# leggedrobotics/delora

Hardware: AMD Instinct MI355X
Metric: training scan-pairs/sec, KITTI 64x2048 range images (higher is better)
Workload: dtype f32; 1 GPU; KITTI-shaped 64x2048, batch=8 pairs/GPU, raw scans of ~141k points (ragged, raster order), steps rotate over 8 distinct HBM-resident batches, online normals, ResNet pose CNN (11.9M params, identity-pretrained state), Adam; BASELINE configs[1]; global_batch=8, parallelism=dp1, cnn=fp32, cnn_impl=hip trunk: fp32 MFMA, fused Winograd F(2x2,3x3) + direct implicit GEMM, channels_last=False, hip_graph=False, distinct_batches=8, priming_steps=8

## Files before the change

### delora_amd/_lib.py

```python
import ctypes
import os

_HERE = os.path.dirname(os.path.abspath(__file__))
LIB_PATH = os.path.join(_HERE, "csrc", "libdelora_hip.so")
ABI_VERSION = 10


class DeloraHipError(RuntimeError):
    pass


class SensorStruct(ctypes.Structure):
    _fields_ = [("H", ctypes.c_int32), ("W", ctypes.c_int32),
                ("hfov0", ctypes.c_double), ("hfov1", ctypes.c_double),
                ("vfov0", ctypes.c_double), ("vfov1", ctypes.c_double)]


_vp, _i32, _i64, _u32, _f32, _sz = (ctypes.c_void_p, ctypes.c_int32, ctypes.c_int64, ctypes.c_uint32,
                                    ctypes.c_float, ctypes.c_size_t)
_SP = ctypes.POINTER(SensorStruct)

SIGNATURES = {
    "dl_abi_version": (_i32, []),
    "dl_last_error": (ctypes.c_char_p, []),
# ... 70 lines not shown
    "dl_heads_single_bwd_workspace_bytes": (_sz, [_i32, _i32, _i32, _i32, _i32, _i32, _i32]),
    "dl_heads_single_bwd": (_i32, [_vp, _vp, _i32, _i32, _i32, _i32, _i32, _i32, _i32, _i32, _vp, _vp, _vp, _vp, _vp, _vp, _vp, _vp, _vp, _vp]),
    "dl_dropout_scale_f32": (_i32, [_vp, _u32, ctypes.c_double, _i64, _vp, _vp]),
    "dl_stem_input_nhwc_drop_f32": (_i32, [_vp, _i32, _i32, _i32, _i32, _vp, ctypes.c_double, _vp, _vp]),
    "dl_channel_scale_nhwc_t": (_i32, [_vp, _vp, _i32, _i32, _i32, _i32, _vp, _vp]),
    "dl_channel_scale_bwd_act_nhwc_t": (_i32, [_vp, _vp, _vp, _i32, _i32, _i32, _i32, _i32, _vp, _vp]),
    "dl_tower_wide_drop_f32": (_i32, [_vp, _vp, ctypes.c_double, _i32, _i32, _i32, _i32, _i32, _vp, _vp]),
    "dl_tower_wide_drop_bwd_f32": (_i32, [_vp, _vp, _vp, ctypes.c_double, _i32, _i32, _i32, _i32, _i32, _i32, _vp, _vp]),
    "dl_mean_hw_nhwc_h": (_i32, [_vp, _i32, _i32, _i32, _i32, _vp, _vp]),
    "dl_mean_hw_bwd_act_h": (_i32, [_vp, _vp, _i32, _i32, _i32, _i32, _i32, _vp, _vp]),
    "dl_conv2d_wgrad_h_workspace_bytes": (_sz, [_i32, _i32, _i32, _i32, _i32, _i32, _i32, _i32]),
    "dl_conv2d_wgrad_nhwc_h": (_i32, [_vp, _vp, _vp, _vp, _i32, _i32, _i32, _i32, _i32, _i32, _i32, _i32, _i32, _vp]),
    "dl_wgrad_batch_plan": (_i64, [_vp, _vp, _i32, _i32, _i32, _vp]),
    "dl_wino_wgrad3x3_batch_workspace_bytes": (_sz, [_vp, _i32]),
    "dl_wino_wgrad3x3_batch_nhwc_f32": (_i32, [_vp, _i32, _vp, _vp]),
    "dl_conv2d_wgrad_batch_workspace_bytes": (_sz, [_vp, _i32]),
    "dl_conv2d_wgrad_batch_nhwc_f32": (_i32, [_vp, _i32, _vp, _vp]),
    "dl_conv2d_wgrad_batch_h_workspace_bytes": (_sz, [_vp, _i32]),
    "dl_conv2d_wgrad_batch_nhwc_h": (_i32, [_vp, _i32, _vp, _i32, _vp]),
    "dl_conv_plan_describe": (_i32, [_i32, _i32, _i32, _i32, _i32, _i32, _i32, _i32, _i32, _i32, _i32, _i32, ctypes.c_char_p, _sz]),
    "dl_pose_net_prepared_bytes": (_sz, [_vp, _i32, _i32, _i32]),
    "dl_pose_net_prepare": (_i32, [_vp, _i32, _i32, _i32, _vp, _vp]),
    "dl_pose_net_workspace_bytes": (_sz, [_vp, _i32, _i32, _i32]),
    "dl_pose_net_forward": (_i32, [_vp, _vp, _vp, _i64, _vp, _i64, _i32, _i32, _i32, _vp, _vp, _vp, _vp, _vp]),
    "dl_odometry_workspace_bytes": (_sz, [_vp, _SP, _i32, _i32, _i32]),
    "dl_odometry_push": (_i32, [_vp, _vp, _SP, _vp, _i64, _i32, _vp, _vp, _vp, _vp, _vp, _vp, _vp, _vp]),
    "dl_profile_begin": (_i32, [_i32, ctypes.c_char_p]),
    "dl_profile_end": (_i32, [_vp, _i32, ctypes.POINTER(ctypes.c_int32), ctypes.POINTER(ctypes.c_int32)]),
    "dl_profile_pause": (_i32, [_i32]),
}
# ... 109 lines not shown
```

### delora_amd/csrc/wino.hip

```cpp
#include "common.h"
#include <cstdlib>

typedef float f32x16 __attribute__((ext_vector_type(16)));
typedef float f32x4 __attribute__((ext_vector_type(4)));
typedef float f32x2 __attribute__((ext_vector_type(2)));
typedef int i32x4 __attribute__((ext_vector_type(4)));

#define WN_THREADS 512
#define WN_CK 8
#define WN_KB 64
#define WN_TILES 64
#define WN_PLANE (WN_TILES * WN_CK + 16)
#define WN_EPI_ADD 1u
#define WN_EPI_ACT 2u
#define WN_EPI_DACT 4u

struct WinoArgs {
  const float* x;
  const float* u;
  float* y;
  const float* add;
  const float* dsrc;
  int N, H, W, C, K;
  int act;
// ... 518 lines not shown
template <bool NEG> __device__ __forceinline__ f32x2 w3_g01(f32x2 h, f32x2 c01) {
  f32x2 r;
  if (NEG) asm volatile("v_pk_fma_f32 %0, %1, %2, %1 op_sel:[1,0,0] op_sel_hi:[1,1,0] neg_lo:[1,0,1] neg_hi:[1,0,1]" : "=v"(r) : "v"(h), "s"(c01));
  else asm volatile("v_pk_fma_f32 %0, %1, %2, %1 op_sel:[1,0,0] op_sel_hi:[1,1,0]" : "=v"(r) : "v"(h), "s"(c01));
  return r;
}
template <bool NEG> __device__ __forceinline__ f32x2 w3_g23(f32x2 h, f32x2 c10) {
  f32x2 r;
  if (NEG) asm volatile("v_pk_fma_f32 %0, %1, %2, %1 op_sel:[0,0,1] op_sel_hi:[0,1,1] neg_lo:[1,0,0] neg_hi:[1,0,0]" : "=v"(r) : "v"(h), "s"(c10));
  else asm volatile("v_pk_fma_f32 %0, %1, %2, %1 op_sel:[0,0,1] op_sel_hi:[0,1,1] neg_lo:[0,0,1] neg_hi:[0,0,1]" : "=v"(r) : "v"(h), "s"(c10));
  return r;
}

struct W3Pos { int n, ta, b8; };

__device__ __forceinline__ void wino_wgrad_body3(const WWArgs& a, const int blk) {
  static_assert((2 * W3_BUF + W3_RAW + W3_GRAW) * 4 <= 163840, "LDS budget");
  __shared__ __attribute__((aligned(16))) float lds[2 * W3_BUF + W3_RAW + W3_GRAW];
  float* raw = lds + 2 * W3_BUF;
  float* graw = raw + W3_RAW;
  const int tid = threadIdx.x, lane = tid & 63, wave = __builtin_amdgcn_readfirstlane(tid >> 6);
  const int li = lane & 31, half = lane >> 5;
  const int mb = wave & 1, nb = (wave >> 1) & 1, xh = wave >> 2;
  const int CT = a.C / 64;
  int t = blk;
  const int slab = t % a.nslabs; t /= a.nslabs;
  const int ct = t % CT;
  const int kt = t / CT;
  const int k0 = kt * 64, c0 = ct * 64;
  const int th = a.H / 2, tw8 = (a.W / 2) / 8;
  const int total_chunks = a.N * th * tw8;
  const int ch_begin = slab * a.chunks_per_slab;
  const int ch_end = min(ch_begin + a.chunks_per_slab, total_chunks);
  if (ch_begin >= ch_end) return;

  const unsigned lds_base = (unsigned)(__SIZE_TYPE__)((__attribute__((address_space(3))) char*)lds);
  const int tp = wave & 3;
#define W3_SWZ(R) ((((R) >> 2) & 1) | (((((R) >> 1) ^ ((R) >> 3)) & 1) << 1))
  const int w_off = lane * 16 + ((tp ^ W3_SWZ(lane)) * 4);
  const float* rsrc = (xh == 0 ? raw : graw) + (4 * tp) * 64 + lane;
  const unsigned voff_x = (unsigned)((lane >> 4) * a.C * 4 + (lane & 15) * 16);
  const unsigned voff_g = (unsigned)((lane >> 4) * a.K * 4 + (lane & 15) * 16);
  const unsigned voff_l = (unsigned)(((lane >> 4) == 0 ? a.W - 1 : (lane >> 4) - 1) * a.C * 4 + (lane & 15) * 16);
  const unsigned voff_r = (unsigned)(((lane >> 4) == 0 ? a.W - 1 : 0) * a.C * 4 + (lane & 15) * 16);
// ... 52 lines not shown
#define W3_DMASK()          { if (top) { _Pragma("unroll") for (int j = 0; j < 6; ++j) P[0][j][0] = 0.f; }                        \
                              if (bot) { _Pragma("unroll") for (int j = 0; j < 6; ++j) P[1][j][1] = 0.f; } }
#define W3_DT(E, RP, B)     { constexpr int o_ = 2 * (E);                                                                           \
                              T[RP][B] = (B) == 0 ? P[RP][o_] - P[RP][o_ + 2] : (B) == 1 ? P[RP][o_ + 1] + P[RP][o_ + 2]               \
                                       : (B) == 2 ? P[RP][o_ + 2] - P[RP][o_ + 1] : P[RP][o_ + 1] - P[RP][o_ + 3]; }
#define W3_DV(E, B)         { V01[E][B] = w3_v01(T[0][B], T[1][B]); V23[E][B] = w3_v23(T[0][B], T[1][B]); }
#define W3_WR(OPER, B)      { f32x4 lo_ = {V01[0][B][0], V01[0][B][1], V01[1][B][0], V01[1][B][1]};                                  \
                              f32x4 hi_ = {V23[0][B][0], V23[0][B][1], V23[1][B][0], V23[1][B][1]};                                  \
                              *reinterpret_cast<f32x4*>(nxt + (OPER) + (B) * W3_PLANE + w_off) = lo_;                                \
                              *reinterpret_cast<f32x4*>(nxt + (OPER) + (4 + (B)) * W3_PLANE + w_off) = hi_; }
#define W3_GLD()            W3_RD2(P[0][0], 0, 16) W3_RD2(P[0][1], 1, 17) W3_RD2(P[0][2], 2, 18) W3_RD2(P[0][3], 3, 19)
#define W3_GH(E)            { T[E][1] = P[0][2 * (E)] + P[0][2 * (E) + 1]; T[E][2] = P[0][2 * (E)] - P[0][2 * (E) + 1]; }
#define W3_GV(E, B)         { if ((B) == 0) { V01[E][0] = w3_g01<false>(P[0][2 * (E)], c01); V23[E][0] = w3_g23<false>(P[0][2 * (E)], c10); }              \
                              else if ((B) == 3) { V01[E][3] = w3_g01<true>(P[0][2 * (E) + 1], c01); V23[E][3] = w3_g23<true>(P[0][2 * (E) + 1], c10); } \
                              else { V01[E][B] = w3_g01<false>(T[E][B], c01); V23[E][B] = w3_g23<false>(T[E][B], c10); } }

#define W3_FR_FROM(HP, BP)                                                                                                \
  {                                                                                                                       \
    av[(HP) & 1] = *reinterpret_cast<const f32x4*>((BP) + ((HP) >> 1) * W3_PLANE + (((HP) & 1) ? a_off1 : a_off0));       \
    bv[(HP) & 1] = *reinterpret_cast<const f32x4*>((BP) + ((HP) >> 1) * W3_PLANE + (((HP) & 1) ? b_off1 : b_off0));       \
  }
#define W3_FR(HP) W3_FR_FROM(HP, cur)
#define W3_M(HP, J, ...)                                                                                                  \
  {                                                                                                                       \
    acc[((J) & 1) * 4 + ((HP) >> 1)] = __builtin_amdgcn_mfma_f32_32x32x2f32(av[(HP) & 1][J], bv[(HP) & 1][J], acc[((J) & 1) * 4 + ((HP) >> 1)], 0, 0, 0); \
    asm volatile("" : "+v"(acc[((J) & 1) * 4 + ((HP) >> 1)]) :: "memory");                                                 \
    __builtin_amdgcn_sched_barrier(0);                                                                                    \
    __VA_ARGS__                                                                                                           \
    __builtin_amdgcn_sched_barrier(0);                                                                                    \
  }
// ... 3 lines not shown
    int u = ch_begin;
    p1.b8 = u % tw8; u /= tw8;
    p1.ta = u % th;
    p1.n = u / th;
  }
  dma(p1);
  asm volatile("s_waitcnt vmcnt(0)" ::: "memory");
  __syncthreads();
  {
    float* nxt = lds;
    const bool top = p1.ta == 0, bot = p1.ta == th - 1;
    if (xh == 0) {
      W3_DLD_0A() W3_DLD_0B() W3_DLD_1A() W3_DLD_1B()
      asm volatile("s_waitcnt lgkmcnt(0)" ::: "memory");
      W3_DMASK()
      W3_DT(0, 0, 0) W3_DT(0, 0, 1) W3_DT(0, 0, 2) W3_DT(0, 0, 3) W3_DT(0, 1, 0) W3_DT(0, 1, 1) W3_DT(0, 1, 2) W3_DT(0, 1, 3)
      W3_DV(0, 0) W3_DV(0, 1) W3_DV(0, 2) W3_DV(0, 3)
      W3_DT(1, 0, 0) W3_DT(1, 0, 1) W3_DT(1, 0, 2) W3_DT(1, 0, 3) W3_DT(1, 1, 0) W3_DT(1, 1, 1) W3_DT(1, 1, 2) W3_DT(1, 1, 3)
      W3_DV(1, 0) W3_DV(1, 1) W3_DV(1, 2) W3_DV(1, 3)
      W3_WR(W3_OPER, 0) W3_WR(W3_OPER, 1) W3_WR(W3_OPER, 2) W3_WR(W3_OPER, 3)
    } else {
      W3_GLD()
      asm volatile("s_waitcnt lgkmcnt(0)" ::: "memory");
      W3_GH(0) W3_GH(1)
      W3_GV(0, 0) W3_GV(0, 1) W3_GV(0, 2) W3_GV(0, 3) W3_GV(1, 0) W3_GV(1, 1) W3_GV(1, 2) W3_GV(1, 3)
      W3_WR(0, 0) W3_WR(0, 1) W3_WR(0, 2) W3_WR(0, 3)
    }
  }
  __syncthreads();
  if (ch_begin + 1 < ch_end) advance(p1);
  dma(p1);
  asm volatile("s_waitcnt vmcnt(0)" ::: "memory");
  __syncthreads();

  f32x4 av[2], bv[2];
  {
    const float* cur = lds;
    W3_FR(0)
  }
#define W3_TAIL()                                                                                                         \
    W3_M(6, 0, W3_FR(7)) W3_M(6, 1, ) W3_M(6, 2, ) W3_M(6, 3, )                                                           \
    asm volatile("s_waitcnt vmcnt(0) lgkmcnt(0)" ::: "memory");                                                           \
    __builtin_amdgcn_s_barrier();                                                                                         \
    __builtin_amdgcn_sched_barrier(0);                                                                                    \
    W3_M(7, 0, W3_FR_FROM(0, nxt)) W3_M(7, 1, ) W3_M(7, 2, ) W3_M(7, 3, )
#define W3_BAR_M()                                                                                                        \
    asm volatile("s_waitcnt lgkmcnt(0)" ::: "memory");                                                                    \
    __builtin_amdgcn_s_barrier();                                                                                         \
    __builtin_amdgcn_sched_barrier(0);
  if (xh == 0) {
    for (int ch = ch_begin; ch < ch_end; ++ch) {
      const float* cur = lds + ((ch - ch_begin) & 1) * W3_BUF;
      float* nxt = lds + ((ch - ch_begin + 1) & 1) * W3_BUF;
      const bool top = p1.ta == 0, bot = p1.ta == th - 1;
      W3Pos p2 = p1;
      if (ch + 2 < ch_end) advance(p2);
      W3_M(0, 0, WW_IF_FR(W3_FR(1)) WW_IF_T(W3_DLD_0A())) W3_M(0, 1, WW_IF_T(W3_DLD_0B())) W3_M(0, 2, WW_IF_T(W3_DLD_1A())) W3_M(0, 3, WW_IF_T(W3_DLD_1B()))
      W3_M(1, 0, WW_IF_FR(W3_FR(2))) W3_M(1, 1, ) W3_M(1, 2, ) W3_M(1, 3, )
      asm volatile("s_waitcnt lgkmcnt(0)" ::: "memory");
      WW_IF_BAR(__builtin_amdgcn_s_barrier();)
      __builtin_amdgcn_sched_barrier(0);
      W3_M(2, 0, WW_IF_FR(W3_FR(3)) WW_IF_DMA(dma(p2);)) W3_M(2, 1, WW_IF_T(W3_DMASK()) WW_IF_T(W3_DT(0, 0, 0)) WW_IF_T(W3_DT(0, 0, 1))) W3_M(2, 2, WW_IF_T(W3_DT(0, 0, 2)) WW_IF_T(W3_DT(0, 0, 3))) W3_M(2, 3, WW_IF_T(W3_DT(0, 1, 0)) WW_IF_T(W3_DT(0, 1, 1)))
      W3_M(3, 0, WW_IF_FR(W3_FR(4)) WW_IF_T(W3_DT(0, 1, 2)) WW_IF_T(W3_DT(0, 1, 3))) W3_M(3, 1, WW_IF_T(W3_DV(0, 0))) W3_M(3, 2, WW_IF_T(W3_DV(0, 1))) W3_M(3, 3, WW_IF_T(W3_DV(0, 2)))
      W3_M(4, 0, WW_IF_FR(W3_FR(5)) WW_IF_T(W3_DV(0, 3))) W3_M(4, 1, WW_IF_T(W3_DT(1, 0, 0)) WW_IF_T(W3_DT(1, 0, 1))) W3_M(4, 2, WW_IF_T(W3_DT(1, 0, 2)) WW_IF_T(W3_DT(1, 0, 3))) W3_M(4, 3, WW_IF_T(W3_DT(1, 1, 0)) WW_IF_T(W3_DT(1, 1, 1)))
      W3_M(5, 0, WW_IF_FR(W3_FR(6)) WW_IF_T(W3_DT(1, 1, 2)) WW_IF_T(W3_DT(1, 1, 3))) W3_M(5, 1, WW_IF_T(W3_DV(1, 0)) WW_IF_T(W3_WR(W3_OPER, 0))) W3_M(5, 2, WW_IF_T(W3_DV(1, 1)) WW_IF_T(W3_WR(W3_OPER, 1))) W3_M(5, 3, WW_IF_T(W3_DV(1, 2)) WW_IF_T(W3_WR(W3_OPER, 2)))
// ... 33 lines not shown
#undef W3_RD2
#undef W3_DLD_0A
#undef W3_DLD_0B
#undef W3_DLD_1A
#undef W3_DLD_1B
#undef W3_DMASK
#undef W3_DT
#undef W3_DV
#undef W3_WR
#undef W3_GLD
#undef W3_GH
#undef W3_GV
#undef W3_FR
#undef W3_FR_FROM
#undef W3_M
  float* wp = a.ws + ((size_t)slab * 16) * a.K * a.C;
#pragma unroll
  for (int xl = 0; xl < 8; ++xl) {
    const int xi = xh * 8 + xl;
#pragma unroll
    for (int q = 0; q < 16; ++q) {
      const int m = mb * 32 + 8 * (q / 4) + 4 * half + (q % 4);
      wp[((size_t)xi * a.K + k0 + m) * a.C + c0 + nb * 32 + li] = acc[xl][q];
    }
  }
}

template <bool RAG>
__global__ __launch_bounds__(WW_THREADS) void k_wino_wgrad(WWArgs a) {
#ifndef WW_OLD
  if constexpr (!RAG) wino_wgrad_body3(a, blockIdx.x);
  else
#endif
  wino_wgrad_body<RAG>(a, blockIdx.x);
}

struct WWBatchArgs {
  WWArgs layer[DL_WGRAD_BATCH];
  int first_wg[DL_WGRAD_BATCH + 1];
  int n;
};
template <bool RAG>
__global__ __launch_bounds__(WW_THREADS) void k_wino_wgrad_batch(WWBatchArgs b) {
  int l = 0;
#pragma unroll
  for (int i = 1; i < DL_WGRAD_BATCH; ++i)
    if (i < b.n && (int)blockIdx.x >= b.first_wg[i]) l = i;
  const WWArgs a = b.layer[l];
#ifndef WW_OLD
  if constexpr (!RAG) wino_wgrad_body3(a, (int)blockIdx.x - b.first_wg[l]);
  else
#endif
  wino_wgrad_body<RAG>(a, (int)blockIdx.x - b.first_wg[l]);
}

__device__ __forceinline__ void wino_wgrad_sum_body(const float* __restrict__ ws, int nslabs, size_t count4, float* __restrict__ u, size_t i) {
  if (i >= count4) return;
  f32x4 s = {0.f, 0.f, 0.f, 0.f};
  for (int sl = 0; sl < nslabs; ++sl) s += reinterpret_cast<const f32x4*>(ws)[(size_t)sl * count4 + i];
  reinterpret_cast<f32x4*>(u)[i] = s;
}
__global__ __launch_bounds__(256) void k_wino_wgrad_sum(const float* __restrict__ ws, int nslabs, size_t count4, float* __restrict__ u) {
  wino_wgrad_sum_body(ws, nslabs, count4, u, (size_t)blockIdx.x * 256 + threadIdx.x);
}

__device__ __forceinline__ void wino_wgrad_out_body(const float* __restrict__ uu, int K, int C, float* __restrict__ dw, size_t i);
__global__ __launch_bounds__(256) void k_wino_wgrad_out(const float* __restrict__ uu, int K, int C, float* __restrict__ dw) {
  wino_wgrad_out_body(uu, K, C, dw, (size_t)blockIdx.x * 256 + threadIdx.x);
// ... 194 lines not shown
    if (it.a.nslabs > 1) {
      sum.src[sum.n] = it.a.ws; sum.dst[sum.n] = it.usum; sum.K[sum.n] = it.a.K; sum.C[sum.n] = it.a.C; sum.nslabs[sum.n] = it.a.nslabs;
      sum.first_block[sum.n] = sum_blocks;
      sum_blocks += (int)(((size_t)16 * it.a.K * it.a.C / 4 + 255) / 256);
      ++sum.n;
    }
    out.src[out.n] = it.usum; out.dst[out.n] = it.dw; out.K[out.n] = it.a.K; out.C[out.n] = it.a.C;
    out.first_block[out.n] = out_blocks;
    out_blocks += (int)(((size_t)it.a.K * it.a.C + 255) / 256);
    ++out.n;
  }
  sum.first_block[sum.n] = sum_blocks; out.first_block[out.n] = out_blocks;
  if (sum.n) DL_LAUNCH_PLAIN(k_wino_wgrad_sum_batch, dim3(sum_blocks), dim3(256), st, sum);
  DL_LAUNCH_PLAIN(k_wino_wgrad_out_batch, dim3(out_blocks), dim3(256), st, out);
  return dl_check_launch("dl_wino_wgrad3x3_batch_nhwc_f32");
}

__global__ __launch_bounds__(256) void k_wino_split_sum(const float* __restrict__ part, int splits, size_t count4, float* __restrict__ y,
                                                         const float* __restrict__ add, const float* __restrict__ dsrc, int act, unsigned epi) {
  const size_t i = (size_t)blockIdx.x * 256 + threadIdx.x;
  if (i >= count4) return;
  const f32x4* p = reinterpret_cast<const f32x4*>(part) + i;
  f32x4 v = p[0];
  for (int s = 1; s < splits; ++s) v += p[(size_t)s * count4];
  if (epi & WN_EPI_ADD) v += reinterpret_cast<const f32x4*>(add)[i];
  if (epi & WN_EPI_ACT) {
    if (act == 1) { v[0] = dl_tanh(v[0]); v[1] = dl_tanh(v[1]); v[2] = dl_tanh(v[2]); v[3] = dl_tanh(v[3]); }
    else { v[0] = wn_act(v[0], act); v[1] = wn_act(v[1], act); v[2] = wn_act(v[2], act); v[3] = wn_act(v[3], act); }
  }
  if (epi & WN_EPI_DACT) {
// ... 193 lines not shown
```

### delora_amd/models/ring_conv.py

```python
import ctypes
import os

import torch

from .. import _lib

ACT = {"none": 0, "tanh": 1, "relu": 2}
USE_WINOGRAD = True
EPI_ADD, EPI_ACT, EPI_DACT, EPI_ADD_GRID = 1, 2, 4, 8


def _ptr(t):
    return ctypes.c_void_p(t.data_ptr()) if t is not None else ctypes.c_void_p(0)


def _stream():
    return ctypes.c_void_p(torch.cuda.current_stream().cuda_stream)


ALLOC_SKEW = 0
_skew_state = {"i": 0}


def _empty(shape, dtype, device):
# ... 76 lines not shown
    lib = _lib.load()
    out = []
    for i0 in range(0, len(items), _lib.WGRAD_BATCH):
        part = items[i0:i0 + _lib.WGRAD_BATCH]
        arr, dws = _wgrad_layer_table(part)
        ap = ctypes.cast(arr, ctypes.c_void_p)
        nbytes = getattr(lib, size_fn)(ap, len(part))
        if not nbytes:
            raise _lib.DeloraHipError(what + ": " + (lib.dl_last_error() or b"").decode())
        ws = torch.empty((nbytes // 4,), dtype=torch.float32, device=part[0][0].device)
        _lib.check(getattr(lib, run_fn)(ap, len(part), _ptr(ws), *extra, _stream()), what)
        out += dws
    return out


def wgrad_batch(items):
    wino, direct = [], []
    for i, (x, g, ks, stride) in enumerate(items):
        N, H, W, C = x.shape
        K = g.shape[3]
        if (USE_WINOGRAD_WGRAD and ks == 3 and tuple(stride) == (1, 1) and C >= WINO_WGRAD_MIN_C_BATCHED and C % 64 == 0 and K % 64 == 0 and W >= 2
                and N * H * W * max(C, K) < 2 ** 31 and H * W * max(C, K) < 2 ** 30):
            wino.append(i)
        else:
            direct.append(i)
    out = [None] * len(items)
    if wino:
        for i, dw in zip(wino, _wgrad_batch_call([items[i] for i in wino], "dl_wino_wgrad3x3_batch_workspace_bytes", "dl_wino_wgrad3x3_batch_nhwc_f32",
                                                 "dl_wino_wgrad3x3_batch_nhwc_f32")):
            out[i] = dw
    if direct:
        for i, dw in zip(direct, _wgrad_batch_call([items[i] for i in direct], "dl_conv2d_wgrad_batch_workspace_bytes", "dl_conv2d_wgrad_batch_nhwc_f32",
                                                   "dl_conv2d_wgrad_batch_nhwc_f32")):
            out[i] = dw
    return out


def wino_ok(H, W, C, K):
    return H >= 1 and W >= 1 and C % 8 == 0 and K % 64 == 0


# ... 844 lines not shown
```

### include/delora_hip.h

```cpp
#ifndef DELORA_HIP_H
#define DELORA_HIP_H

#include <stddef.h>
#include <stdint.h>

#ifdef __cplusplus
extern "C" {
#endif

#define DL_ABI_VERSION 10

typedef void* dl_stream;

typedef enum {
  DL_OK = 0,
  DL_ERR_INVALID_ARGUMENT = -1,
  DL_ERR_LAUNCH = -2,
  DL_ERR_UNSUPPORTED = -3
} dl_status;

typedef struct {
  int32_t H;
  int32_t W;
  double hfov0, hfov1;
// ... 146 lines not shown
int dl_wino_wgrad3x3_nhwc_f32(const float* x, const float* g, float* dw, void* workspace, int32_t N, int32_t H, int32_t W,
                              int32_t C, int32_t K, dl_stream stream);

#define DL_WGRAD_BATCH 24
typedef struct dl_wgrad_layer {
  const void* x;
  const void* g;
  float* dw;
  int32_t N, H, W, C, K, ksize, stride_h, stride_w;
} dl_wgrad_layer;
int64_t dl_wgrad_batch_plan(const int32_t* tiles, const int32_t* chunks, int32_t n, int32_t slots, int32_t partial_cost, int32_t* nslabs);
size_t dl_wino_wgrad3x3_batch_workspace_bytes(const dl_wgrad_layer* layers, int32_t n);
int dl_wino_wgrad3x3_batch_nhwc_f32(const dl_wgrad_layer* layers, int32_t n, void* workspace, dl_stream stream);
size_t dl_conv2d_wgrad_batch_workspace_bytes(const dl_wgrad_layer* layers, int32_t n);
int dl_conv2d_wgrad_batch_nhwc_f32(const dl_wgrad_layer* layers, int32_t n, void* workspace, dl_stream stream);

int dl_conv_weights_h(const float* w, void* w_fwd, void* w_bwd, int32_t K, int32_t taps, int32_t C, int32_t dtype, dl_stream stream);
#define DL_CONVH_BATCH 32
typedef struct {
  const float* w;
  void* w_fwd;
  void* w_bwd;
  int32_t K, taps, C;
} dl_convh_layer;
int dl_conv_weights_batch_h(const dl_convh_layer* layers, int32_t n, int32_t dtype, dl_stream stream);
int dl_conv2d_nhwc_h(const void* x, const void* w, void* y, const void* add, const void* dsrc, int32_t N, int32_t H, int32_t W,
                     int32_t C, int32_t K, int32_t ksize, int32_t stride_h, int32_t stride_w, int32_t transposed, int32_t dtype,
                     int32_t act, uint32_t epilogue, dl_stream stream);
int dl_conv2d_dgrad_strided_nhwc_h(const void* g, const void* w, void* dx, const void* add_grid, const void* dsrc, int32_t N,
                                   int32_t H, int32_t W, int32_t K, int32_t C, int32_t ksize, int32_t stride_h, int32_t stride_w,
// ... 127 lines not shown
```

Before: 693.6 scan-pairs/s.

## Add Winograd weight-gradient path for stride-(1,2) 3x3 convolutions via column polyphase split

Adds a batched Winograd F(2x2,3x3) weight-gradient kernel for 3x3 convolutions with stride (1,2). The input is treated as two interleaved polyphase halves of width W/2 and 2C channels, and only the live Winograd column sets are computed (three for the odd phase, two for the even phase). A templated body skips the dead columns with its own MFMA/transform schedules, followed by a slab-sum kernel and an output kernel that folds the two phases back into 3x3 filter taps. Python routes eligible strided layers to this path instead of the direct implicit-GEMM wgrad, aiming to cut MFMA work and memory traffic. The cost is extra workspace, an extra reduction/combine launch and more code complexity.

```diff
diff --git a/delora_amd/_lib.py b/delora_amd/_lib.py
--- a/delora_amd/_lib.py
+++ b/delora_amd/_lib.py
@@ -108,6 +108,9 @@
     "dl_wgrad_batch_plan": (_i64, [_vp, _vp, _i32, _i32, _i32, _vp]),
     "dl_wino_wgrad3x3_batch_workspace_bytes": (_sz, [_vp, _i32]),
     "dl_wino_wgrad3x3_batch_nhwc_f32": (_i32, [_vp, _i32, _vp, _vp]),
+    "dl_wino_strided_wgrad_takes": (_i32, [_i32, _i32, _i32, _i32, _i32, _i32, _i32]),
+    "dl_wino_strided_wgrad3x3_batch_workspace_bytes": (_sz, [_vp, _i32]),
+    "dl_wino_strided_wgrad3x3_batch_nhwc_f32": (_i32, [_vp, _i32, _vp, _vp]),
     "dl_conv2d_wgrad_batch_workspace_bytes": (_sz, [_vp, _i32]),
     "dl_conv2d_wgrad_batch_nhwc_f32": (_i32, [_vp, _i32, _vp, _vp]),
     "dl_conv2d_wgrad_batch_h_workspace_bytes": (_sz, [_vp, _i32]),
diff --git a/delora_amd/csrc/wino.hip b/delora_amd/csrc/wino.hip
--- a/delora_amd/csrc/wino.hip
+++ b/delora_amd/csrc/wino.hip
@@ -556,20 +556,23 @@
 
 struct W3Pos { int n, ta, b8; };
 
-__device__ __forceinline__ void wino_wgrad_body3(const WWArgs& a, const int blk) {
-  static_assert((2 * W3_BUF + W3_RAW + W3_GRAW) * 4 <= 163840, "LDS budget");
-  __shared__ __attribute__((aligned(16))) float lds[2 * W3_BUF + W3_RAW + W3_GRAW];
+static_assert((2 * W3_BUF + W3_RAW + W3_GRAW) * 4 <= 163840, "LDS budget");
+__shared__ __attribute__((aligned(16))) float w3_lds[2 * W3_BUF + W3_RAW + W3_GRAW];
+template <int LIVE, bool UPPER = LIVE == 0x7>
+__device__ __forceinline__ void wino_wgrad_body3_live(const WWArgs& a, const int blk) {
+  static_assert(LIVE == 0xF || LIVE == 0x7 || LIVE == 0x6, "column sets with a schedule");
+  float* const lds = w3_lds;
   float* raw = lds + 2 * W3_BUF;
   float* graw = raw + W3_RAW;
   const int tid = threadIdx.x, lane = tid & 63, wave = __builtin_amdgcn_readfirstlane(tid >> 6);
   const int li = lane & 31, half = lane >> 5;
   const int mb = wave & 1, nb = (wave >> 1) & 1, xh = wave >> 2;
-  const int CT = a.C / 64;
+  const int CT = LIVE == 0xF ? a.C / 64 : a.C / 128;
   int t = blk;
   const int slab = t % a.nslabs; t /= a.nslabs;
   const int ct = t % CT;
   const int kt = t / CT;
-  const int k0 = kt * 64, c0 = ct * 64;
+  const int k0 = kt * 64, c0 = ct * 64 + (UPPER ? a.C / 2 : 0);
   const int th = a.H / 2, tw8 = (a.W / 2) / 8;
   const int total_chunks = a.N * th * tw8;
   const int ch_begin = slab * a.chunks_per_slab;
@@ -652,6 +655,13 @@
 #define W3_GV(E, B)         { if ((B) == 0) { V01[E][0] = w3_g01<false>(P[0][2 * (E)], c01); V23[E][0] = w3_g23<false>(P[0][2 * (E)], c10); }              \
                               else if ((B) == 3) { V01[E][3] = w3_g01<true>(P[0][2 * (E) + 1], c01); V23[E][3] = w3_g23<true>(P[0][2 * (E) + 1], c10); } \
                               else { V01[E][B] = w3_g01<false>(T[E][B], c01); V23[E][B] = w3_g23<false>(T[E][B], c10); } }
+#define W3_B(B, ...)        { if constexpr ((LIVE >> (B)) & 1) { __VA_ARGS__ } }
+#define W3_DLD7_0A() W3_RD2(P[0][0], 0, 20) W3_RD2(P[0][1], 1, 21) W3_RD2(P[0][2], 2, 22)
+#define W3_DLD7_1A() W3_RD2(P[1][0], 40, 60) W3_RD2(P[1][1], 41, 61) W3_RD2(P[1][2], 42, 62)
+#define W3_DLD6_0A() W3_RD2(P[0][1], 1, 21) W3_RD2(P[0][2], 2, 22)
+#define W3_DLD6_1A() W3_RD2(P[1][1], 41, 61) W3_RD2(P[1][2], 42, 62)
+#define W3_DLDL_0B() W3_RD2(P[0][3], 3, 23) W3_RD2(P[0][4], 4, 24)
+#define W3_DLDL_1B() W3_RD2(P[1][3], 43, 63) W3_RD2(P[1][4], 44, 64)
 
 #define W3_FR_FROM(HP, BP)                                                                                                \
   {                                                                                                                       \
@@ -685,17 +695,20 @@
       W3_DLD_0A() W3_DLD_0B() W3_DLD_1A() W3_DLD_1B()
       asm volatile("s_waitcnt lgkmcnt(0)" ::: "memory");
       W3_DMASK()
-      W3_DT(0, 0, 0) W3_DT(0, 0, 1) W3_DT(0, 0, 2) W3_DT(0, 0, 3) W3_DT(0, 1, 0) W3_DT(0, 1, 1) W3_DT(0, 1, 2) W3_DT(0, 1, 3)
-      W3_DV(0, 0) W3_DV(0, 1) W3_DV(0, 2) W3_DV(0, 3)
-      W3_DT(1, 0, 0) W3_DT(1, 0, 1) W3_DT(1, 0, 2) W3_DT(1, 0, 3) W3_DT(1, 1, 0) W3_DT(1, 1, 1) W3_DT(1, 1, 2) W3_DT(1, 1, 3)
-      W3_DV(1, 0) W3_DV(1, 1) W3_DV(1, 2) W3_DV(1, 3)
-      W3_WR(W3_OPER, 0) W3_WR(W3_OPER, 1) W3_WR(W3_OPER, 2) W3_WR(W3_OPER, 3)
+      W3_B(0, W3_DT(0, 0, 0)) W3_B(1, W3_DT(0, 0, 1)) W3_B(2, W3_DT(0, 0, 2)) W3_B(3, W3_DT(0, 0, 3))
+      W3_B(0, W3_DT(0, 1, 0)) W3_B(1, W3_DT(0, 1, 1)) W3_B(2, W3_DT(0, 1, 2)) W3_B(3, W3_DT(0, 1, 3))
+      W3_B(0, W3_DV(0, 0)) W3_B(1, W3_DV(0, 1)) W3_B(2, W3_DV(0, 2)) W3_B(3, W3_DV(0, 3))
+      W3_B(0, W3_DT(1, 0, 0)) W3_B(1, W3_DT(1, 0, 1)) W3_B(2, W3_DT(1, 0, 2)) W3_B(3, W3_DT(1, 0, 3))
+      W3_B(0, W3_DT(1, 1, 0)) W3_B(1, W3_DT(1, 1, 1)) W3_B(2, W3_DT(1, 1, 2)) W3_B(3, W3_DT(1, 1, 3))
+      W3_B(0, W3_DV(1, 0)) W3_B(1, W3_DV(1, 1)) W3_B(2, W3_DV(1, 2)) W3_B(3, W3_DV(1, 3))
+      W3_B(0, W3_WR(W3_OPER, 0)) W3_B(1, W3_WR(W3_OPER, 1)) W3_B(2, W3_WR(W3_OPER, 2)) W3_B(3, W3_WR(W3_OPER, 3))
     } else {
       W3_GLD()
       asm volatile("s_waitcnt lgkmcnt(0)" ::: "memory");
       W3_GH(0) W3_GH(1)
-      W3_GV(0, 0) W3_GV(0, 1) W3_GV(0, 2) W3_GV(0, 3) W3_GV(1, 0) W3_GV(1, 1) W3_GV(1, 2) W3_GV(1, 3)
-      W3_WR(0, 0) W3_WR(0, 1) W3_WR(0, 2) W3_WR(0, 3)
+      W3_B(0, W3_GV(0, 0)) W3_B(1, W3_GV(0, 1)) W3_B(2, W3_GV(0, 2)) W3_B(3, W3_GV(0, 3))
+      W3_B(0, W3_GV(1, 0)) W3_B(1, W3_GV(1, 1)) W3_B(2, W3_GV(1, 2)) W3_B(3, W3_GV(1, 3))
+      W3_B(0, W3_WR(0, 0)) W3_B(1, W3_WR(0, 1)) W3_B(2, W3_WR(0, 2)) W3_B(3, W3_WR(0, 3))
     }
   }
   __syncthreads();
@@ -704,10 +717,11 @@
   asm volatile("s_waitcnt vmcnt(0)" ::: "memory");
   __syncthreads();
 
+  constexpr int HP0 = LIVE & 1 ? 0 : 2;
   f32x4 av[2], bv[2];
   {
     const float* cur = lds;
-    W3_FR(0)
+    W3_FR(HP0)
   }
 #define W3_TAIL()                                                                                                         \
     W3_M(6, 0, W3_FR(7)) W3_M(6, 1, ) W3_M(6, 2, ) W3_M(6, 3, )                                                           \
@@ -719,7 +733,81 @@
     asm volatile("s_waitcnt lgkmcnt(0)" ::: "memory");                                                                    \
     __builtin_amdgcn_s_barrier();                                                                                         \
     __builtin_amdgcn_sched_barrier(0);
-  if (xh == 0) {
+#define W3_BAR_E()                                                                                                        \
+    asm volatile("s_waitcnt vmcnt(0) lgkmcnt(0)" ::: "memory");                                                           \
+    __builtin_amdgcn_s_barrier();                                                                                         \
+    __builtin_amdgcn_sched_barrier(0);
+  if constexpr (LIVE != 0xF) {
+    if (xh == 0) { if constexpr (LIVE == 0x7) { W3_DLD7_0A() W3_DLD7_1A() } else { W3_DLD6_0A() W3_DLD6_1A() } W3_DLDL_0B() W3_DLDL_1B() }
+    else { W3_GLD() }
+  }
+  if constexpr (LIVE == 0x7) {
+    if (xh == 0) {
+      for (int ch = ch_begin; ch < ch_end; ++ch) {
+        const float* cur = lds + ((ch - ch_begin) & 1) * W3_BUF;
+        float* nxt = lds + ((ch - ch_begin + 1) & 1) * W3_BUF;
+        const bool top = p1.ta == 0, bot = p1.ta == th - 1;
+        W3Pos p2 = p1;
+        if (ch + 2 < ch_end) advance(p2);
+        W3_BAR_M()
+        W3_M(0, 0, W3_FR(1) dma(p2);) W3_M(0, 1, W3_DMASK() W3_DT(0, 0, 0) W3_DT(0, 0, 1)) W3_M(0, 2, W3_DT(0, 0, 2) W3_DT(0, 1, 0)) W3_M(0, 3, W3_DT(0, 1, 1) W3_DT(0, 1, 2))
+        W3_M(1, 0, W3_FR(2) W3_DV(0, 0)) W3_M(1, 1, W3_DV(0, 1)) W3_M(1, 2, W3_DV(0, 2)) W3_M(1, 3, W3_DT(1, 0, 0) W3_DT(1, 0, 1))
+        W3_M(2, 0, W3_FR(3) W3_DT(1, 0, 2)) W3_M(2, 1, W3_DT(1, 1, 0) W3_DT(1, 1, 1)) W3_M(2, 2, W3_DT(1, 1, 2)) W3_M(2, 3, W3_DV(1, 0))
+        W3_M(3, 0, W3_FR(4) W3_WR(W3_OPER, 0)) W3_M(3, 1, W3_DV(1, 1)) W3_M(3, 2, W3_WR(W3_OPER, 1)) W3_M(3, 3, W3_DV(1, 2))
+        W3_M(4, 0, W3_FR(5) W3_WR(W3_OPER, 2)) W3_M(4, 1, ) W3_M(4, 2, ) W3_M(4, 3, )
+        W3_BAR_E()
+        W3_M(5, 0, W3_FR_FROM(0, nxt) W3_DLD7_0A() W3_DLDL_0B()) W3_M(5, 1, W3_DLD7_1A() W3_DLDL_1B()) W3_M(5, 2, ) W3_M(5, 3, )
+        p1 = p2;
+      }
+    } else {
+      for (int ch = ch_begin; ch < ch_end; ++ch) {
+        const float* cur = lds + ((ch - ch_begin) & 1) * W3_BUF;
+        float* nxt = lds + ((ch - ch_begin + 1) & 1) * W3_BUF;
+        W3Pos p2 = p1;
+        if (ch + 2 < ch_end) advance(p2);
+        W3_BAR_M()
+        W3_M(0, 0, W3_FR(1) dma(p2);) W3_M(0, 1, W3_GH(0)) W3_M(0, 2, W3_GV(0, 0)) W3_M(0, 3, W3_GV(0, 1))
+        W3_M(1, 0, W3_FR(2)) W3_M(1, 1, W3_GV(0, 2)) W3_M(1, 2, W3_GH(1)) W3_M(1, 3, W3_GV(1, 0))
+        W3_M(2, 0, W3_FR(3) W3_WR(0, 0)) W3_M(2, 1, W3_GV(1, 1)) W3_M(2, 2, W3_WR(0, 1)) W3_M(2, 3, W3_GV(1, 2))
+        W3_M(3, 0, W3_FR(4) W3_WR(0, 2)) W3_M(3, 1, ) W3_M(3, 2, ) W3_M(3, 3, )
+        W3_M(4, 0, W3_FR(5)) W3_M(4, 1, ) W3_M(4, 2, ) W3_M(4, 3, )
+        W3_BAR_E()
+        W3_M(5, 0, W3_FR_FROM(0, nxt) W3_GLD()) W3_M(5, 1, ) W3_M(5, 2, ) W3_M(5, 3, )
+        p1 = p2;
+      }
+    }
+  } else if constexpr (LIVE == 0x6) {
+    if (xh == 0) {
+      for (int ch = ch_begin; ch < ch_end; ++ch) {
+        const float* cur = lds + ((ch - ch_begin) & 1) * W3_BUF;
+        float* nxt = lds + ((ch - ch_begin + 1) & 1) * W3_BUF;
+        const bool top = p1.ta == 0, bot = p1.ta == th - 1;
+        W3Pos p2 = p1;
+        if (ch + 2 < ch_end) advance(p2);
+        W3_BAR_M()
+        W3_M(2, 0, W3_FR(3) dma(p2);) W3_M(2, 1, W3_DMASK() W3_DT(0, 0, 1) W3_DT(0, 0, 2)) W3_M(2, 2, W3_DT(0, 1, 1) W3_DT(0, 1, 2)) W3_M(2, 3, W3_DV(0, 1))
+        W3_M(3, 0, W3_FR(4) W3_DV(0, 2)) W3_M(3, 1, W3_DT(1, 0, 1) W3_DT(1, 0, 2)) W3_M(3, 2, W3_DT(1, 1, 1) W3_DT(1, 1, 2)) W3_M(3, 3, W3_DV(1, 1))
+        W3_M(4, 0, W3_FR(5) W3_WR(W3_OPER, 1)) W3_M(4, 1, W3_DV(1, 2)) W3_M(4, 2, W3_WR(W3_OPER, 2)) W3_M(4, 3, )
+        W3_BAR_E()
+        W3_M(5, 0, W3_FR_FROM(2, nxt) W3_DLD6_0A() W3_DLDL_0B()) W3_M(5, 1, W3_DLD6_1A() W3_DLDL_1B()) W3_M(5, 2, ) W3_M(5, 3, )
+        p1 = p2;
+      }
+    } else {
+      for (int ch = ch_begin; ch < ch_end; ++ch) {
+        const float* cur = lds + ((ch - ch_begin) & 1) * W3_BUF;
+        float* nxt = lds + ((ch - ch_begin + 1) & 1) * W3_BUF;
+        W3Pos p2 = p1;
+        if (ch + 2 < ch_end) advance(p2);
+        W3_BAR_M()
+        W3_M(2, 0, W3_FR(3) dma(p2);) W3_M(2, 1, W3_GH(0)) W3_M(2, 2, W3_GV(0, 1)) W3_M(2, 3, W3_GV(0, 2))
+        W3_M(3, 0, W3_FR(4)) W3_M(3, 1, W3_GH(1)) W3_M(3, 2, W3_GV(1, 1)) W3_M(3, 3, W3_GV(1, 2))
+        W3_M(4, 0, W3_FR(5) W3_WR(0, 1)) W3_M(4, 1, W3_WR(0, 2)) W3_M(4, 2, ) W3_M(4, 3, )
+        W3_BAR_E()
+        W3_M(5, 0, W3_FR_FROM(2, nxt) W3_GLD()) W3_M(5, 1, ) W3_M(5, 2, ) W3_M(5, 3, )
+        p1 = p2;
+      }
+    }
+  } else if (xh == 0) {
     for (int ch = ch_begin; ch < ch_end; ++ch) {
       const float* cur = lds + ((ch - ch_begin) & 1) * W3_BUF;
       float* nxt = lds + ((ch - ch_begin + 1) & 1) * W3_BUF;
@@ -783,17 +871,47 @@
 #undef W3_FR
 #undef W3_FR_FROM
 #undef W3_M
-  float* wp = a.ws + ((size_t)slab * 16) * a.K * a.C;
-#pragma unroll
-  for (int xl = 0; xl < 8; ++xl) {
-    const int xi = xh * 8 + xl;
-#pragma unroll
-    for (int q = 0; q < 16; ++q) {
-      const int m = mb * 32 + 8 * (q / 4) + 4 * half + (q % 4);
-      wp[((size_t)xi * a.K + k0 + m) * a.C + c0 + nb * 32 + li] = acc[xl][q];
-    }
-  }
-}
+#undef W3_B
+#undef W3_BAR_E
+#undef W3_DLD7_0A
+#undef W3_DLD7_1A
+#undef W3_DLD6_0A
+#undef W3_DLD6_1A
+#undef W3_DLDL_0B
+#undef W3_DLDL_1B
+  if constexpr (LIVE == 0xF) {
+    float* wp = a.ws + ((size_t)slab * 16) * a.K * a.C;
+#pragma unroll
+    for (int xl = 0; xl < 8; ++xl) {
+      const int xi = xh * 8 + xl;
+#pragma unroll
+      for (int q = 0; q < 16; ++q) {
+        const int m = mb * 32 + 8 * (q / 4) + 4 * half + (q % 4);
+        wp[((size_t)xi * a.K + k0 + m) * a.C + c0 + nb * 32 + li] = acc[xl][q];
+      }
+    }
+  } else {
+    constexpr int NB = (LIVE & 1) + ((LIVE >> 1) & 1) + ((LIVE >> 2) & 1) + ((LIVE >> 3) & 1);
+    const int CL = a.C / 2, cl0 = c0 >= CL ? c0 - CL : c0;
+    float* wp = a.ws + ((size_t)slab * 4 * NB) * a.K * CL;
+#pragma unroll
+    for (int xl = 0; xl < 8; ++xl) {
+      const int b = xl & 3;
+      if (!((LIVE >> b) & 1)) continue;
+      int bi = 0;
+#pragma unroll
+      for (int j = 0; j < 4; ++j) bi += (j < b && ((LIVE >> j) & 1)) ? 1 : 0;
+      const int plane = (xh * 2 + (xl >> 2)) * NB + bi;
+#pragma unroll
+      for (int q = 0; q < 16; ++q) {
+        const int m = mb * 32 + 8 * (q / 4) + 4 * half + (q % 4);
+        wp[((size_t)plane * a.K + k0 + m) * CL + cl0 + nb * 32 + li] = acc[xl][q];
+      }
+    }
+  }
+}
+
+__device__ __forceinline__ void wino_wgrad_body3(const WWArgs& a, const int blk) { wino_wgrad_body3_live<0xF>(a, blk); }
 
 template <bool RAG>
 __global__ __launch_bounds__(WW_THREADS) void k_wino_wgrad(WWArgs a) {
@@ -821,6 +939,25 @@
   else
 #endif
   wino_wgrad_body<RAG>(a, (int)blockIdx.x - b.first_wg[l]);
+}
+
+#define SW_ITEMS (2 * DL_WGRAD_BATCH)
+struct SWBatchArgs {
+  WWArgs item[SW_ITEMS];
+  int first_wg[SW_ITEMS + 1];
+  int odd[SW_ITEMS];
+  int n;
+};
+template <bool ALL12>
+__global__ __launch_bounds__(WW_THREADS) void k_wino_wgrad_strided_batch(SWBatchArgs b) {
+  int l = 0;
+#pragma unroll
+  for (int i = 1; i < SW_ITEMS; ++i)
+    if (i < b.n && (int)blockIdx.x >= b.first_wg[i]) l = i;
+  const WWArgs a = b.item[l];
+  if (b.odd[l]) wino_wgrad_body3_live<0x7>(a, (int)blockIdx.x - b.first_wg[l]);
+  else if constexpr (ALL12) wino_wgrad_body3_live<0x7, false>(a, (int)blockIdx.x - b.first_wg[l]);
+  else wino_wgrad_body3_live<0x6>(a, (int)blockIdx.x - b.first_wg[l]);
 }
 
 __device__ __forceinline__ void wino_wgrad_sum_body(const float* __restrict__ ws, int nslabs, size_t count4, float* __restrict__ u, size_t i) {
@@ -1045,6 +1182,194 @@
   if (sum.n) DL_LAUNCH_PLAIN(k_wino_wgrad_sum_batch, dim3(sum_blocks), dim3(256), st, sum);
   DL_LAUNCH_PLAIN(k_wino_wgrad_out_batch, dim3(out_blocks), dim3(256), st, out);
   return dl_check_launch("dl_wino_wgrad3x3_batch_nhwc_f32");
+}
+
+struct SWSumArgs {
+  const float* src[SW_ITEMS];
+  float* dst[SW_ITEMS];
+  int count4[SW_ITEMS], nslabs[SW_ITEMS];
+  int first_block[SW_ITEMS + 1];
+  int n;
+};
+__global__ __launch_bounds__(256) void k_wino_wgrad_strided_sum_batch(SWSumArgs b) {
+  int l = 0;
+#pragma unroll
+  for (int i = 1; i < SW_ITEMS; ++i)
+    if (i < b.n && (int)blockIdx.x >= b.first_block[i]) l = i;
+  wino_wgrad_sum_body(b.src[l], b.nslabs[l], (size_t)b.count4[l], b.dst[l], (size_t)((int)blockIdx.x - b.first_block[l]) * 256 + threadIdx.x);
+}
+struct SWOutArgs {
+  const float* uo[DL_WGRAD_BATCH];
+  const float* ue[DL_WGRAD_BATCH];
+  float* dw[DL_WGRAD_BATCH];
+  int K[DL_WGRAD_BATCH], C[DL_WGRAD_BATCH];
+  int first_block[DL_WGRAD_BATCH + 1];
+  int n, eb;
+};
+__device__ __forceinline__ float sw_gt(int rr, float u0, float u1, float u2, float u3) {
+  return rr == 0 ? u0 + 0.5f * (u1 + u2) : rr == 1 ? 0.5f * (u1 - u2) : 0.5f * (u1 + u2) + u3;
+}
+__global__ __launch_bounds__(256) void k_wino_wgrad_strided_out_batch(SWOutArgs b) {
+  int l = 0;
+#pragma unroll
+  for (int i = 1; i < DL_WGRAD_BATCH; ++i)
+    if (i < b.n && (int)blockIdx.x >= b.first_block[i]) l = i;
+  const int K = b.K[l], C = b.C[l];
+  const size_t i = (size_t)((int)blockIdx.x - b.first_block[l]) * 256 + threadIdx.x;
+  if (i >= (size_t)K * C) return;
+  const int k = (int)(i / C), c = (int)(i % C);
+  const float* __restrict__ uo = b.uo[l];
+  const float* __restrict__ ue = b.ue[l];
+  float* __restrict__ dw = b.dw[l];
+  float o[4][3], e[4][2];
+#pragma unroll
+  for (int a = 0; a < 4; ++a) {
+#pragma unroll
+    for (int j = 0; j < 3; ++j) o[a][j] = uo[((size_t)(a * 3 + j) * K + k) * C + c];
+#pragma unroll
+    for (int j = 0; j < 2; ++j) e[a][j] = ue[((size_t)(a * b.eb + b.eb - 2 + j) * K + k) * C + c];
+  }
+#pragma unroll
+  for (int rr = 0; rr < 3; ++rr) {
+    const float p0 = sw_gt(rr, o[0][0], o[1][0], o[2][0], o[3][0]);
+    const float p1 = sw_gt(rr, o[0][1], o[1][1], o[2][1], o[3][1]);
+    const float p2 = sw_gt(rr, o[0][2], o[1][2], o[2][2], o[3][2]);
+    const float q1 = sw_gt(rr, e[0][0], e[1][0], e[2][0], e[3][0]);
+    const float q2 = sw_gt(rr, e[0][1], e[1][1], e[2][1], e[3][1]);
+    dw[(((size_t)k * 3 + rr) * 3 + 0) * C + c] = p0 + 0.5f * (p1 + p2);
+    dw[(((size_t)k * 3 + rr) * 3 + 1) * C + c] = 0.5f * (q1 - q2);
+    dw[(((size_t)k * 3 + rr) * 3 + 2) * C + c] = 0.5f * (p1 - p2);
+  }
+}
+
+static bool sw_takes(int N, int H, int W, int C, int K, int sh, int sw) {
+  return sh == 1 && sw == 2 && N > 0 && H > 0 && W > 0 && C > 0 && K > 0 && !(H & 1) && W % 32 == 0 && C % 64 == 0 && K % 64 == 0 &&
+         ww_supported(N, H, W / 2, 2 * C, K);
+}
+extern "C" int dl_wino_strided_wgrad_takes(int32_t N, int32_t H, int32_t W, int32_t C, int32_t K, int32_t stride_h, int32_t stride_w) {
+  return sw_takes(N, H, W, C, K, stride_h, stride_w) ? 1 : 0;
+}
+
+namespace {
+struct SWItem {
+  WWArgs a;
+  float* usum;
+  int odd, layer, tiles, planes;
+};
+bool sw_all12() {
+  static const bool on = [] { const char* e = getenv("DL_SWGRAD_ALL12"); return e && e[0] == '1'; }();
+  return on;
+}
+int sw_batch_plan(const dl_wgrad_layer* L, int n, std::vector<SWItem>& items) {
+  const char* me = "dl_wino_strided_wgrad3x3_batch_nhwc_f32";
+  if (!L || n <= 0 || n > DL_WGRAD_BATCH) return dl_fail(DL_ERR_INVALID_ARGUMENT, "%s: 1..%d layers per call", me, DL_WGRAD_BATCH);
+  for (int i = 0; i < n; ++i) {
+    const dl_wgrad_layer& l = L[i];
+    if (l.ksize != 3) return dl_fail(DL_ERR_UNSUPPORTED, "%s: layer %d: ksize %d (must be 3)", me, i, l.ksize);
+    if (l.stride_h != 1 || l.stride_w != 2) return dl_fail(DL_ERR_UNSUPPORTED, "%s: layer %d: stride_h, stride_w (%d,%d) (must be (1,2))", me, i, l.stride_h, l.stride_w);
+    if (l.H <= 0 || (l.H & 1)) return dl_fail(DL_ERR_UNSUPPORTED, "%s: layer %d: H %d (must be even)", me, i, l.H);
+    if (l.W <= 0 || l.W % 32) return dl_fail(DL_ERR_UNSUPPORTED, "%s: layer %d: W %d (must be a multiple of 32)", me, i, l.W);
+    if (l.C <= 0 || l.C % 64) return dl_fail(DL_ERR_UNSUPPORTED, "%s: layer %d: C %d (must be a multiple of 64)", me, i, l.C);
+    if (l.K <= 0 || l.K % 64) return dl_fail(DL_ERR_UNSUPPORTED, "%s: layer %d: K %d (must be a multiple of 64)", me, i, l.K);
+    if (!sw_takes(l.N, l.H, l.W, l.C, l.K, 1, 2))
+      return dl_fail(DL_ERR_UNSUPPORTED, "%s: layer %d: N %d with H=%d W=%d C=%d K=%d (positive, below 2^31 elements and 2^30 per sample)", me, i, l.N, l.H, l.W, l.C, l.K);
+  }
+  items.resize(2 * n);
+  std::vector<int> tl(2 * n), ch(2 * n), ns(2 * n);
+  for (int i = 0; i < n; ++i) {
+    const dl_wgrad_layer& l = L[i];
+    const int chunks = l.N * (l.H / 2) * (l.W / 32);
+    for (int odd = 1; odd >= 0; --odd) {
+      SWItem& it = items[2 * i + (1 - odd)];
+      it.a = WWArgs{(const float*)l.x, (const float*)l.g, nullptr, l.N, l.H, l.W / 2, 2 * l.C, l.K, 0, 0};
+      it.usum = nullptr; it.odd = odd; it.layer = i;
+      it.tiles = (l.K / 64) * (l.C / 64);
+      it.planes = odd || sw_all12() ? 12 : 8;
+      tl[2 * i + (1 - odd)] = it.tiles;
+      ch[2 * i + (1 - odd)] = it.planes == 12 ? chunks : (3 * chunks + 3) / 4;
+    }
+  }
+  dl_plan_batch(tl.data(), ch.data(), 2 * n, 256, 10, ns.data());
+  for (int j = 0; j < 2 * n; ++j) {
+    SWItem& it = items[j];
+    const int chunks = it.a.N * (it.a.H / 2) * (it.a.W / 16);
+    const int want = ns[j] < chunks ? ns[j] : chunks;
+    it.a.chunks_per_slab = (chunks + want - 1) / want;
+    it.a.nslabs = (chunks + it.a.chunks_per_slab - 1) / it.a.chunks_per_slab;
+  }
+  return DL_OK;
+}
+}
+
+extern "C" size_t dl_wino_strided_wgrad3x3_batch_workspace_bytes(const dl_wgrad_layer* layers, int32_t n) {
+  std::vector<SWItem> items;
+  if (sw_batch_plan(layers, n, items)) return 0;
+  size_t floats = 0;
+  for (const auto& it : items) floats += ((size_t)(it.a.nslabs > 1 ? it.a.nslabs : 0) + 1) * it.planes * it.a.K * (it.a.C / 2);
+  return floats * sizeof(float);
+}
+
+extern "C" int dl_wino_strided_wgrad3x3_batch_nhwc_f32(const dl_wgrad_layer* layers, int32_t n, void* workspace, dl_stream stream) {
+  if (!workspace) return dl_fail(DL_ERR_INVALID_ARGUMENT, "dl_wino_strided_wgrad3x3_batch_nhwc_f32: null workspace");
+  std::vector<SWItem> items;
+  const int rc0 = sw_batch_plan(layers, n, items);
+  if (rc0) return rc0;
+  for (int i = 0; i < n; ++i)
+    if (!layers[i].x || !layers[i].g || !layers[i].dw) return dl_fail(DL_ERR_INVALID_ARGUMENT, "dl_wino_strided_wgrad3x3_batch_nhwc_f32: layer %d: null pointer", i);
+  hipStream_t st = (hipStream_t)stream;
+  float* wsf = (float*)workspace;
+  for (auto& it : items) {
+    const size_t plane = (size_t)it.planes * it.a.K * (it.a.C / 2);
+    if (it.a.nslabs > 1) { it.a.ws = wsf; wsf += (size_t)it.a.nslabs * plane; it.usum = wsf; wsf += plane; }
+    else { it.a.ws = wsf; it.usum = wsf; wsf += plane; }
+  }
+  std::vector<const SWItem*> grp;
+  for (const auto& it : items) grp.push_back(&it);
+  std::stable_sort(grp.begin(), grp.end(), [](const SWItem* x, const SWItem* y) {
+    return x->a.chunks_per_slab * (x->planes / 4 + 1) > y->a.chunks_per_slab * (y->planes / 4 + 1);
+  });
+  SWBatchArgs b{};
+  b.n = (int)grp.size();
+  int wgs = 0;
+  double flop = 0, bytes = 0;
+  for (int i = 0; i < b.n; ++i) {
+    const WWArgs& a = grp[i]->a;
+    b.item[i] = a;
+    b.odd[i] = grp[i]->odd;
+    b.first_wg[i] = wgs;
+    wgs += grp[i]->tiles * a.nslabs;
+    flop += 2.0 * grp[i]->planes * (double)a.N * (a.H / 2) * (a.W / 2) * 64.0 * 64.0 * grp[i]->tiles;
+    if (grp[i]->odd) bytes += 4.0 * ((double)a.N * a.H * a.W * (a.C + a.K) + 9.0 * (a.C / 2) * a.K);
+  }
+  b.first_wg[b.n] = wgs;
+  const dl_wgrad_layer& f = layers[grp[0]->layer];
+  const DlProfTag tag{"k_wino_wgrad_strided", n > 1 ? "wgrad-batch" : "wgrad", f.N, f.H, f.W, f.C, f.K, 3, 1, 2, flop, bytes};
+  if (sw_all12()) DL_LAUNCH(tag, k_wino_wgrad_strided_batch<true>, dim3(wgs), dim3(WW_THREADS), st, b);
+  else DL_LAUNCH(tag, k_wino_wgrad_strided_batch<false>, dim3(wgs), dim3(WW_THREADS), st, b);
+  for (int i = 0; i < b.n; ++i) DL_PLAN_NOTE("%s slabs=%d", b.odd[i] ? "odd" : "even", b.item[i].nslabs);
+  SWSumArgs sum{};
+  SWOutArgs out{};
+  int sum_blocks = 0, out_blocks = 0;
+  for (const auto& it : items) {
+    if (it.a.nslabs > 1) {
+      const size_t count4 = (size_t)it.planes * it.a.K * (it.a.C / 2) / 4;
+      sum.src[sum.n] = it.a.ws; sum.dst[sum.n] = it.usum; sum.count4[sum.n] = (int)count4; sum.nslabs[sum.n] = it.a.nslabs;
+      sum.first_block[sum.n] = sum_blocks;
+      sum_blocks += (int)((count4 + 255) / 256);
+      ++sum.n;
+    }
+    if (it.odd) out.uo[it.layer] = it.usum; else out.ue[it.layer] = it.usum;
+  }
+  for (int i = 0; i < n; ++i) {
+    out.dw[i] = layers[i].dw; out.K[i] = layers[i].K; out.C[i] = layers[i].C;
+    out.first_block[i] = out_blocks;
+    out_blocks += (int)(((size_t)layers[i].K * layers[i].C + 255) / 256);
+  }
+  out.n = n; out.eb = sw_all12() ? 3 : 2;
+  sum.first_block[sum.n] = sum_blocks; out.first_block[n] = out_blocks;
+  if (sum.n) DL_LAUNCH_PLAIN(k_wino_wgrad_strided_sum_batch, dim3(sum_blocks), dim3(256), st, sum);
+  DL_LAUNCH_PLAIN(k_wino_wgrad_strided_out_batch, dim3(out_blocks), dim3(256), st, out);
+  return dl_check_launch("dl_wino_strided_wgrad3x3_batch_nhwc_f32");
 }
 
 __global__ __launch_bounds__(256) void k_wino_split_sum(const float* __restrict__ part, int splits, size_t count4, float* __restrict__ y,
diff --git a/delora_amd/models/ring_conv.py b/delora_amd/models/ring_conv.py
--- a/delora_amd/models/ring_conv.py
+++ b/delora_amd/models/ring_conv.py
@@ -114,17 +114,35 @@
     return out
 
 
+USE_WINOGRAD_STRIDED_WGRAD = True
+WINO_STRIDED_WGRAD_MIN_CHUNKS = 256
+
+
+def wino_strided_wgrad_ok(N, H, W, C, K, stride):
+    if tuple(stride) != (1, 2) or min(N, H, W, C, K) <= 0 or H % 2 or W % 32 or C % 64 or K % 64:
+        return False
+    wide = max(2 * C, K)
+    return N * H * (W // 2) * wide < 2 ** 31 and H * (W // 2) * wide < 2 ** 30
+
+
 def wgrad_batch(items):
-    wino, direct = [], []
+    wino, strided, direct = [], [], []
     for i, (x, g, ks, stride) in enumerate(items):
         N, H, W, C = x.shape
         K = g.shape[3]
         if (USE_WINOGRAD_WGRAD and ks == 3 and tuple(stride) == (1, 1) and C >= WINO_WGRAD_MIN_C_BATCHED and C % 64 == 0 and K % 64 == 0 and W >= 2
                 and N * H * W * max(C, K) < 2 ** 31 and H * W * max(C, K) < 2 ** 30):
             wino.append(i)
+        elif (USE_WINOGRAD and USE_WINOGRAD_STRIDED_WGRAD and ks == 3 and wino_strided_wgrad_ok(N, H, W, C, K, stride)
+                and N * (H // 2) * (W // 32) >= WINO_STRIDED_WGRAD_MIN_CHUNKS):
+            strided.append(i)
         else:
             direct.append(i)
     out = [None] * len(items)
+    if strided:
+        for i, dw in zip(strided, _wgrad_batch_call([items[i] for i in strided], "dl_wino_strided_wgrad3x3_batch_workspace_bytes",
+                                                    "dl_wino_strided_wgrad3x3_batch_nhwc_f32", "dl_wino_strided_wgrad3x3_batch_nhwc_f32")):
+            out[i] = dw
     if wino:
         for i, dw in zip(wino, _wgrad_batch_call([items[i] for i in wino], "dl_wino_wgrad3x3_batch_workspace_bytes", "dl_wino_wgrad3x3_batch_nhwc_f32",
                                                  "dl_wino_wgrad3x3_batch_nhwc_f32")):
diff --git a/include/delora_hip.h b/include/delora_hip.h
--- a/include/delora_hip.h
+++ b/include/delora_hip.h
@@ -184,6 +184,9 @@
 int dl_wino_wgrad3x3_batch_nhwc_f32(const dl_wgrad_layer* layers, int32_t n, void* workspace, dl_stream stream);
 size_t dl_conv2d_wgrad_batch_workspace_bytes(const dl_wgrad_layer* layers, int32_t n);
 int dl_conv2d_wgrad_batch_nhwc_f32(const dl_wgrad_layer* layers, int32_t n, void* workspace, dl_stream stream);
+int dl_wino_strided_wgrad_takes(int32_t N, int32_t H, int32_t W, int32_t C, int32_t K, int32_t stride_h, int32_t stride_w);
+size_t dl_wino_strided_wgrad3x3_batch_workspace_bytes(const dl_wgrad_layer* layers, int32_t n);
+int dl_wino_strided_wgrad3x3_batch_nhwc_f32(const dl_wgrad_layer* layers, int32_t n, void* workspace, dl_stream stream);
 
 int dl_conv_weights_h(const float* w, void* w_fwd, void* w_bwd, int32_t K, int32_t taps, int32_t C, int32_t dtype, dl_stream stream);
 #define DL_CONVH_BATCH 32
```

Result: faster. 703.2 scan-pairs/s (median of 6 runs) (+1.4%).
